# alanross/AlvaAR

Hardware: AMD Instinct MI355X
Metric: frames/sec @640x480 2000kp; local-BA residuals/sec (20KFx3k pts) (higher is better)
Workload: dtype u8/i16 image stages, f32 KLT, f64 pose+BA; 1 GPU; configs[1]: 640x480 RGBA stream, ~2000 keypoints/frame (cell 12), System::findCameraPose dataflow (fb-KLT -> P3P-LMedS -> PnP; keyframes: detect + describe, triangulate, map matching, local BA) via alva_system_find_camera_pose_device, steady state, frames resident in HBM; parallelism=1 independent camera streams, one per GPU, no collective on the data path

## Files before the change

alvaar_amd/csrc/image.hip:

```cpp
#include "common.hpp"
#include "multi_kernel.hpp"

namespace {

__device__ __forceinline__ uint32_t gray_of(uint32_t rgba) {
    uint32_t r = rgba & 0xff, g = (rgba >> 8) & 0xff, b = (rgba >> 16) & 0xff;
    return (9798u * r + 19235u * g + 3735u * b + 16384u) >> 15;
}

__device__ __forceinline__ void store_mirrors(uint8_t *g, size_t pitch, int w, int h, int win, int x, int y, uint8_t v) {
    int xs[3], ys[3];
    int nx = 0, ny = 0;
    xs[nx++] = x;
    if (x >= 1 && x <= win) xs[nx++] = -x;
    if (x <= w - 2 && x >= w - 1 - win) xs[nx++] = 2 * (w - 1) - x;
    ys[ny++] = y;
    if (y >= 1 && y <= win) ys[ny++] = -y;
    if (y <= h - 2 && y >= h - 1 - win) ys[ny++] = 2 * (h - 1) - y;
    if (nx == 1 && ny == 1) return;
    for (int j = 0; j < ny; j++)
        for (int i = 0; i < nx; i++)
            if (i | j) g[(ptrdiff_t) ys[j] * (ptrdiff_t) pitch + xs[i]] = v;
}

template<bool SRC_RGBA>
__device__ __forceinline__ void level0_body(const uint8_t *__restrict__ src, size_t src_pitch, int w, int h, int win,
                                            uint8_t *__restrict__ dst, size_t dst_pitch, uint8_t *__restrict__ gray_out,
                                            size_t gray_out_pitch, const int bx, const int by) {
    int x4 = (bx * 64 + threadIdx.x) * 4;
    int y = by * 4 + threadIdx.y;
    if (x4 >= w || y >= h) return;
    uint32_t packed;
    if (SRC_RGBA) {
        const uint4 p = *reinterpret_cast<const uint4 *>(src + (size_t) y * src_pitch + (size_t) x4 * 4);
        packed = gray_of(p.x) | (gray_of(p.y) << 8) | (gray_of(p.z) << 16) | (gray_of(p.w) << 24);
    } else {
        packed = *reinterpret_cast<const uint32_t *>(src + (size_t) y * src_pitch + x4);
    }
    *reinterpret_cast<uint32_t *>(dst + (size_t) y * dst_pitch + x4) = packed;
    if (gray_out) *reinterpret_cast<uint32_t *>(gray_out + (size_t) y * gray_out_pitch + x4) = packed;
// ... 108 lines not shown
    int acc[4] = {0, 0, 0, 0};
#pragma unroll
    for (int j = 0; j < 5; j++) {
        const uint8_t *row = a.g + (ptrdiff_t) (2 * y - 2 + j) * (ptrdiff_t) a.g_pitch + (2 * x - 4);
        const uint32_t *rp = reinterpret_cast<const uint32_t *>(row);
        const uint32_t w[4] = {rp[0], rp[1], rp[2], rp[3]};
        auto px = [&](int c) -> int { return (int) ((w[c >> 2] >> (8 * (c & 3))) & 0xffu); };
        const int wj = (j == 0 || j == 4) ? 1 : (j == 2 ? 6 : 4);
#pragma unroll
        for (int k = 0; k < 4; k++) {
            const int c0 = 2 + 2 * k;
            const int s = px(c0) + px(c0 + 4) + 4 * (px(c0 + 1) + px(c0 + 3)) + 6 * px(c0 + 2);
            acc[k] += wj * s;
        }
    }
    uint8_t out[4];
#pragma unroll
    for (int k = 0; k < 4; k++) out[k] = (uint8_t) ((acc[k] + 128) >> 8);
    uint8_t *dst = a.ng + (size_t) y * a.ng_pitch + x;
    if (x + 3 < a.dw) {
        *reinterpret_cast<uint32_t *>(dst) = (uint32_t) out[0] | ((uint32_t) out[1] << 8) | ((uint32_t) out[2] << 16) | ((uint32_t) out[3] << 24);
    } else {
        for (int k = 0; k < 4 && x + k < a.dw; k++) dst[k] = out[k];
    }
    for (int k = 0; k < 4 && x + k < a.dw; k++) store_mirrors(a.ng, a.ng_pitch, a.dw, a.dh, a.win, x + k, y, out[k]);
}

__host__ __device__ constexpr int rest_tile(int L) { return L == 3 ? 8 : 16; }
constexpr int R3 = 18;
constexpr int R2 = 23;
constexpr int R1 = 49;
constexpr int R0 = 101;
constexpr int R0P = (R0 + 3 + 3) / 4 * 4;
struct RestLevel {
    uint8_t *g;
    size_t g_pitch;
    int16_t *d;
    size_t d_pitch;
    int w, h;
};
struct RestArgs {
    StageArgs s0;
    RestLevel lv[4];
    int nlevels, win;
    int first[4], bx[4], ntiles[4];
    int ts[4];
};
struct Span {
    int lo, hi;
};
__device__ __forceinline__ int mirror101(int c, int n) { return c < 0 ? -c : (c >= n ? 2 * (n - 1) - c : c); }
__device__ __forceinline__ int mirror_in(int c, int n) { return min(max(mirror101(c, n), 0), n - 1); }
__device__ __forceinline__ Span below(Span s, int n) { return Span{2 * max(s.lo, 0) - 2, 2 * min(s.hi, n - 1) + 2}; }

__device__ __forceinline__ void down_tile(const uint8_t *src, int spitch, Span sx, Span sy, uint8_t *dst, int dpitch, Span dx, Span dy, int nx,
                                          int ny, int tid) {
    const int dw = dx.hi - dx.lo + 1, dh = dy.hi - dy.lo + 1;
    for (int e = tid; e < dw * dh; e += 256) {
        const int j = e / dw, i = e - j * dw;
        const int mx = mirror101(dx.lo + i, nx), my = mirror101(dy.lo + j, ny);
        const uint8_t *p = src + (2 * my - 2 - sy.lo) * spitch + (2 * mx - 2 - sx.lo);
        int acc = 0;
#pragma unroll
        for (int r = 0; r < 5; r++) {
            const uint8_t *q = p + r * spitch;
            const int srow = q[0] + q[4] + 4 * (q[1] + q[3]) + 6 * q[2];
            acc += ((r == 0 || r == 4) ? 1 : (r == 2 ? 6 : 4)) * srow;
        }
        dst[j * dpitch + i] = (uint8_t) ((acc + 128) >> 8);
    }
}

template<bool FROM_RGBA>
__device__ __forceinline__ void deep_tile(const RestArgs &A, int L, int bid, const uint8_t *__restrict__ rgba = nullptr, size_t rgba_pitch = 0) {
    __shared__ __attribute__((aligned(16))) uint8_t b0[R0 * R0P];
    __shared__ uint8_t b1[R1 * R1], b2[R2 * R2], b3[R3 * R3];
    const int tid = threadIdx.y * 64 + threadIdx.x;
    const RestLevel &T = A.lv[L];
    const int ts = A.ts[L];
    const int ox = (bid % A.bx[L]) * ts, oy = (bid / A.bx[L]) * ts;
    __shared__ Span sx[4], sy[4];
    if (tid == 0) {
        sx[L] = Span{ox - 1, min(ox + ts, T.w)};
        sy[L] = Span{oy - 1, min(oy + ts, T.h)};
        for (int l = L; l >= 1; l--) {
            sx[l - 1] = below(sx[l], A.lv[l].w);
            sy[l - 1] = below(sy[l], A.lv[l].h);
        }
    }
    __syncthreads();
    const RestLevel &Z = A.lv[0];
    const int xa = (sx[0].lo & ~3);
    const int ndw = (sx[0].hi - xa) / 4 + 1, nrow = sy[0].hi - sy[0].lo + 1;
    for (int e = tid; e < ndw * nrow; e += 256) {
        const int r = e / ndw, c = e - r * ndw;
        uint32_t v;
        if (FROM_RGBA) {
            const int yy = mirror_in(sy[0].lo + r, Z.h), x0 = xa + 4 * c;
            const uint8_t *rowp = rgba + (size_t) yy * rgba_pitch;
            if (x0 >= 0 && x0 + 3 < Z.w) {
                const uint4 p = *reinterpret_cast<const uint4 *>(rowp + 4 * (size_t) x0);
                v = gray_of(p.x) | (gray_of(p.y) << 8) | (gray_of(p.z) << 16) | (gray_of(p.w) << 24);
            } else {
                v = 0;
#pragma unroll
                for (int k = 0; k < 4; k++)
                    v |= gray_of(*reinterpret_cast<const uint32_t *>(rowp + 4 * (size_t) mirror_in(x0 + k, Z.w))) << (8 * k);
            }
        } else {
            v = *reinterpret_cast<const uint32_t *>(Z.g + (ptrdiff_t) (sy[0].lo + r) * (ptrdiff_t) Z.g_pitch + xa + 4 * c);
        }
        *reinterpret_cast<uint32_t *>(b0 + r * R0P + 4 * c) = v;
    }
    __syncthreads();
    const Span s0x{xa, sx[0].hi};
    Span px = s0x, py = sy[0];
    for (int l = 1; l <= L; l++) {
        const uint8_t *src = l == 1 ? b0 : (l == 2 ? b1 : b2);
        const int sp = l == 1 ? R0P : (l == 2 ? R1 : R2);
        uint8_t *dst = l == L ? b3 : (l == 1 ? b1 : b2);
        const int dp = l == L ? R3 : (l == 1 ? R1 : R2);
        down_tile(src, sp, px, py, dst, dp, sx[l], sy[l], A.lv[l].w, A.lv[l].h, tid);
        __syncthreads();
        px = sx[l];
        py = sy[l];
    }
    const int tx = tid % ts, ty = tid / ts;
    const int x = ox + tx, y = oy + ty;
    if (ty >= ts || x >= T.w || y >= T.h) return;
    const uint8_t *c = b3 + (ty + 1) * R3 + (tx + 1);
    const uint8_t v = c[0];
    T.g[(size_t) y * T.g_pitch + x] = v;
    store_mirrors(T.g, T.g_pitch, T.w, T.h, A.win, x, y, v);
    int t0[3], t1[3];
#pragma unroll
    for (int k = 0; k < 3; k++) {
        const int p0 = c[-R3 + k - 1], p1 = c[k - 1], p2 = c[R3 + k - 1];
        t0[k] = (p0 + p2) * 3 + p1 * 10;
        t1[k] = p2 - p0;
    }
    const short ix = (short) (t0[2] - t0[0]), iy = (short) ((t1[2] + t1[0]) * 3 + t1[1] * 10);
    int16_t *drow = reinterpret_cast<int16_t *>(reinterpret_cast<uint8_t *>(T.d) + (size_t) y * T.d_pitch) + 2 * x;
    *reinterpret_cast<uint32_t *>(drow) = (uint32_t) (uint16_t) ix | ((uint32_t) (uint16_t) iy << 16);
}

__device__ __forceinline__ void pyr_rest_body(const RestArgs &A, const int bid) {
    if (bid < A.s0.scharr_blocks) {
        scharr_tile(A.s0, bid);
        return;
    }
    int L = 1;
    while (L + 1 < A.nlevels && bid >= A.first[L + 1]) L++;
    const int n = A.ntiles[L];
    const int lb = bid - A.first[L], per = (n + 7) / 8;
    const int tile = (lb & 7) * per + (lb >> 3);
    if (tile >= n) return;
    deep_tile<false>(A, L, tile);
}
__global__ void __launch_bounds__(256) k_pyr_rest(RestArgs A) { pyr_rest_body(A, (int) blockIdx.x); }
ALVA_MULTI_KERNEL(MK_PYR_REST, k_pyr_rest_multi, RestArgs, dim3(64, 4), 256, pyr_rest_body(A, bx));

static int all_tile(int L, size_t pixels) {
    if (L == 3) return pixels <= 500000 ? 4 : 6;
    return L == 1 ? 16 : 12;
}
constexpr int L0_TW = 64, L0_TH = 16, L0_P = L0_TW + 8;
struct AllArgs {
    RestArgs R;
    const uint8_t *rgba;
    size_t rgba_pitch;
    uint8_t *gray_out;
    size_t gray_out_pitch;
    int l0_first, l0_bx;
};
__device__ __forceinline__ uint32_t gray4(const uint8_t *p) {
    const uint4 q = *reinterpret_cast<const uint4 *>(p);
    return gray_of(q.x) | (gray_of(q.y) << 8) | (gray_of(q.z) << 16) | (gray_of(q.w) << 24);
}
__device__ __forceinline__ void level0_tile(const AllArgs &A, const int tile) {
    __shared__ __attribute__((aligned(16))) uint8_t t[(L0_TH + 2) * L0_P];
    const int tid = threadIdx.y * 64 + threadIdx.x;
    const RestLevel &Z = A.R.lv[0];
    const int w = Z.w, h = Z.h, win = A.R.win;
    const int ox = (tile % A.l0_bx) * L0_TW, oy = (tile / A.l0_bx) * L0_TH;
    const int tx = tid & 15, ty = tid >> 4;
    const int x4 = ox + 4 * tx, y = oy + ty;
    const bool in = x4 < w && y < h;
    if (in) {
        const uint32_t packed = gray4(A.rgba + (size_t) y * A.rgba_pitch + (size_t) x4 * 4);
        *reinterpret_cast<uint32_t *>(t + (ty + 1) * L0_P + 4 + 4 * tx) = packed;
        *reinterpret_cast<uint32_t *>(Z.g + (size_t) y * Z.g_pitch + x4) = packed;
        if (A.gray_out) *reinterpret_cast<uint32_t *>(A.gray_out + (size_t) y * A.gray_out_pitch + x4) = packed;
        const bool edge_y = (y <= win) || (y >= h - 1 - win);
        const bool edge_x = (x4 <= win) || (x4 + 3 >= w - 1 - win);
        if (edge_x || edge_y) {
#pragma unroll
            for (int k = 0; k < 4; k++) store_mirrors(Z.g, Z.g_pitch, w, h, win, x4 + k, y, (uint8_t) (packed >> (8 * k)));
// ... 344 lines not shown
```

alvaar_amd/csrc/slam/frontend.cpp:

```cpp
#include "slam.hpp"
#if defined(__x86_64__)
#include <immintrin.h>
#endif
#include <chrono>
#include <cstdio>
#include <cmath>
#include <cstdlib>
#include <cstring>
#include <stdexcept>

namespace alva_slam {

namespace {
struct Section {
    double &acc;
    std::chrono::steady_clock::time_point t0 = std::chrono::steady_clock::now();
    explicit Section(double &a) : acc(a) {}
    ~Section() { acc += std::chrono::duration<double>(std::chrono::steady_clock::now() - t0).count(); }
};
}

Slam::Slam(Stages *stages, const Camera &c, const Settings &s) : st(stages), cam(c), cfg(s) {
    const float cw = std::ceil((float) cam.width / (float) cfg.cell_size), ch = std::ceil((float) cam.height / (float) cfg.cell_size);
    cfg.max_keypoints = (int) (cw * ch);
    camera_inverse_K(cam, invK);
    cur = std::make_shared<FrameRec>();
    cur->init(&cam, (size_t) cfg.cell_size);
    st->image_width_ = cam.width;
    st->image_height_ = cam.height;
    ba_arena_.assign((size_t) 4 << 20, 0);
    const char *chk = std::getenv("ALVA_CHECK_OBS_MIRROR");
    check_obs_mirror_ = chk && chk[0] == '1';
    const char *chk_carry = std::getenv("ALVA_CHECK_CARRY");
    check_carry_ = chk_carry && chk_carry[0] == '1';
}

void Slam::reset() {
    slots_dirty_ = true;
    cur->reset();
    st->reset_images();
    pose_failed = 0;
    next_mp_id = next_kf_id = n_map_points = n_keyframes = 0;
    map_generation++;
    keyframes.clear();
    for (auto e: map_points) destroy_map_point(e.second);
    map_points.clear();
    kf_flat_.clear();
    mp_flat_.clear();
    mp_rec_.clear();
    mp_slot_.clear();
    mp_nobs_.clear();
    mp_index_.clear();
    shared_ids.clear();
    ready_for_init = false;
    reset_requested = false;
    lost = false;
    reloc_lost_frames = 0;
}

int Slam::process_frame(const uint8_t *rgba, double timestamp, bool frame_on_device) {
    err_ = 0;
    cur->id++;
    cur->timestamp = timestamp;
    if (lost) return process_lost(rgba, timestamp, frame_on_device);
    track(rgba, timestamp, frame_on_device);
    fail(st->frame_done());
    if (err_) return err_;
    if (reset_requested) {
        reset();
        return 2;
    }
    if (!ready_for_init) return 3;
    if (lost) {
        cur->set_Twc(last_good_Twc_);
        return 4;
    }
    last_good_Twc_ = cur->Twc;
    return 1;
}

void Slam::enter_lost() {
    lost = true;
    reloc_lost_frames = 1;
    reloc_repack_ = true;
    reset_frame();
}
// ... 731 lines not shown
```

alvaar_amd/csrc/slam/map.cpp:

```cpp
#include "slam.hpp"
#if defined(__linux__)
#include <sys/mman.h>
#endif
#include <chrono>
#include <cmath>
#include <cstdio>
#include <cstdlib>
#include <cstring>
#include <limits>
#include <stdexcept>

namespace alva_slam {

namespace {
struct Lap {
    std::chrono::steady_clock::time_point t0 = std::chrono::steady_clock::now();
    void operator()(double &acc) {
        const auto t1 = std::chrono::steady_clock::now();
        acc += std::chrono::duration<double>(t1 - t0).count();
        t0 = t1;
    }
};
}

// ... 246 lines not shown
    if ((int) cur->n_kps > cfg.max_keypoints) {
        for (size_t ci = 0; ci < cur->grid.size(); ci++) {
            if (cur->grid[ci].size() <= 2) continue;
            const std::vector<int> ids = cur->grid[ci].to_vector();
            if (ids.size() > 2) {
                int to_remove = -1;
                size_t min_obs = std::numeric_limits<size_t>::max();
                bool broke = false;
                for (int lmid: ids) {
                    const MpRec *it = rec_raw(lmid);
                    if (it) {
                        const size_t nobs = it->n_obs;
                        if (nobs < min_obs) {
                            to_remove = lmid;
                            min_obs = nobs;
                        }
                    } else {
                        remove_obs_from_cur(lmid);
                        broke = true;
                        break;
                    }
                }
                (void) broke;
                if (to_remove >= 0) remove_obs_from_cur(to_remove);
            }
        }
    }
    ids_scratch_.clear();
    for (const auto &e: cur->kps)
        if (!rec_raw(e.first)) ids_scratch_.push_back(e.first);
    for (int id: ids_scratch_) remove_obs_from_cur(id);
}

void Slam::prepare_frame_observers() {
    const std::vector<int> &ids = kp_ids_;
    for (size_t i = 0; i < ids.size(); i++) {
        const int id = ids[i];
        prefetch_mp(ids.data(), i, ids.size());
        MpRec *r = rec_raw(id);
        if (!r) continue;
        ObsEnt *e = rec_slot(*r, next_kf_id);
        if (!e) {
            med_log.overflow = true;
            continue;
        }
        if (!(e->flags & MPF_OBS)) {
            e->flags |= MPF_OBS;
            r->n_obs++;
        }
        mp_nobs_[(size_t) id] = r->n_obs;
    }
}

void Slam::describe_tracked_begin() {
    const int n = (int) cur->kps.size();
    kp_ids_.clear();
    kp_pts_.resize((size_t) n * 2);
    kp_nodes_.resize((size_t) n);
    size_t i = 0;
    for (auto e: cur->kps) {
        kp_ids_.push_back(e.first);
        kp_nodes_[i] = &e.second;
        kp_pts_[2 * i] = e.second.px[0];
        kp_pts_[2 * i + 1] = e.second.px[1];
        i++;
    }
    if (n) fail(st->describe_begin(n, kp_pts_.data()));
}

void Slam::extract_keypoints() {
    if (err_) return;
    const int n = (int) kp_ids_.size();
    const std::vector<int> &kp_ids = kp_ids_;
    const std::vector<float> &pts = kp_pts_;
    const std::vector<KeyPt *> &nodes = kp_nodes_;
    const int to_detect = cfg.max_keypoints - (int) cur->n_occupied;
    const int cap = (int) cur->grid_cells + 8;
    std::vector<uint8_t> desc((size_t) n * 32), valid((size_t) n);
    if (n) {
        Lap lap;
        if (fail(st->describe_end(desc.data(), valid.data()))) return;
        lap(t_kf[1]);
    }
    Lap lap_det;
    if (to_detect > 0 && fail(st->detect_begin(cfg.cell_size, n, pts.data(), cap))) return;
    lap_det(t_kf[2]);
    if (n) {
        Lap lap;
        for (int i = 0; i < n; i++) {
            prefetch_mp_desc(kp_ids.data(), (size_t) i, (size_t) n);
            if (valid[(size_t) i]) {
                Desc d;
                __builtin_memcpy(d.b, &desc[(size_t) i * 32], 32);
                nodes[(size_t) i]->desc = d;
                nodes[(size_t) i]->has_desc = true;
                MapPt *mp = mp_raw(kp_ids[(size_t) i]);
                if (!mp) throw std::out_of_range("map point");
                mp->add_desc(cur->kfid, d);
            }
        }
        lap(t_kf[15]);
    }
    if (to_detect > 0) {
        std::vector<float> np((size_t) cap * 2);
        int count = 0;
        Lap lap;
        if (fail(st->detect_end(np.data(), &count))) return;
        lap(t_kf[2]);
        if (count > 0) {
            std::vector<uint8_t> desc((size_t) count * 32), valid((size_t) count);
            std::vector<float> unpx((size_t) count * 2);
            std::vector<double> bv((size_t) count * 3);
            if (fail(st->describe_and_compute(count, np.data(), desc.data(), valid.data(), unpx.data(), bv.data()))) return;
            lap(t_kf[3]);
            Lap fine;
            t_fine[26] += (double) count;
            for (int i = 0; i < count; i++) {
                KeyPt k;
                k.id = next_mp_id;
                k.px[0] = np[2 * (size_t) i]; k.px[1] = np[2 * (size_t) i + 1];
                k.unpx[0] = unpx[2 * (size_t) i]; k.unpx[1] = unpx[2 * (size_t) i + 1];
                for (int c = 0; c < 3; c++) k.bv[c] = bv[3 * (size_t) i + c];
                if (valid[(size_t) i]) {
                    __builtin_memcpy(k.desc.b, &desc[(size_t) i * 32], 32);
                    k.has_desc = true;
                    cur->add(k);
                    add_map_point(&k.desc);
                } else {
                    cur->add(k);
                    add_map_point(nullptr);
                }
            }
            fine(t_fine[13]);
        }
    }
}

void *alva_huge_alloc(size_t bytes) {
    const size_t huge = (size_t) 2 << 20, sz = (bytes + huge - 1) / huge * huge;
    void *p = std::aligned_alloc(huge, sz);
    if (!p) return nullptr;
#if defined(__linux__)
    static const bool off = std::getenv("ALVA_NO_HUGE_ARENA") != nullptr;
    if (!off) madvise(p, sz, MADV_HUGEPAGE);
#endif
    std::memset(p, 0, sz);
    return p;
}

Slam::~Slam() {
    if (chunk_ahead_.th.joinable()) chunk_ahead_.th.join();
}

void Slam::start_chunk_ahead(int index) {
    static const bool off = std::getenv("ALVA_NO_CHUNK_AHEAD") != nullptr;
    if (off || chunk_ahead_.th.joinable()) return;
    chunk_ahead_.index = index;
    chunk_ahead_.rec = nullptr;
    chunk_ahead_.dsc.reset();
    chunk_ahead_.keys.reset();
    chunk_ahead_.objs.reset();
    chunk_ahead_.th = std::thread([this, index] {
        chunk_ahead_.rec = st->mp_arena_chunk(index);
        chunk_ahead_.dsc = HugeArray<DescBlock>(MP_CHUNK);
// ... 25 lines not shown
        if (!dsc) dsc = HugeArray<DescBlock>(MP_CHUNK);
        if (!keys) keys = HugeArray<DescKeys>(MP_CHUNK);
        if (!objs) objs = HugeArray<MapPtBox>(MP_CHUNK);
        if (!dsc || !keys || !objs) return false;
        med_log.chunks.push_back(chunk);
        med_log.desc_chunks.push_back(std::move(dsc));
        med_log.key_chunks.push_back(std::move(keys));
        mp_obj_chunks_.push_back(std::move(objs));
        static const bool timing = std::getenv("ALVA_ARENA_TIMING") != nullptr;
        if (timing)
            std::fprintf(stderr, "[arena] chunk %d: %.0f us\n", index, 1e6 * std::chrono::duration<double>(std::chrono::steady_clock::now() - t0).count());
        start_chunk_ahead(index + 1);
    }
    return true;
}

const ObsEnt *Slam::obs_of(const MapPt &mp, int kfid) const {
    const ObsEnt *o = mp.in_kf(kfid);
    if (check_obs_mirror_) {
        const FrameRec *kf = kf_raw(kfid);
        const KeyPt *kp = kf ? kf->find(mp.id()) : nullptr;
        if ((kp != nullptr) != (o != nullptr) || (kp && (std::memcmp(kp->px, o->px, 8) || std::memcmp(kp->unpx, o->unpx, 8)))) {
            std::fprintf(stderr, "alva_slam: observation mirror out of sync (map point %d, keyframe %d)\n", mp.id(), kfid);
            std::abort();
        }
    }
    return o;
}

void Slam::add_keyframe() {
    Lap fine;
    std::shared_ptr<FrameRec> kf = std::make_shared<FrameRec>(*cur);
    fine(t_fine[10]);
    for (const auto &e: kf->kps) {
        MapPt *m = mp_raw(e.first);
        if (m) m->note_px(next_kf_id, e.second);
    }
    fine(t_fine[12]);
    keyframes.emplace(next_kf_id, kf);
    if (kf_flat_.size() <= (size_t) next_kf_id) kf_flat_.resize((size_t) next_kf_id + 32, nullptr);
    kf_flat_[(size_t) next_kf_id] = kf.get();
    n_keyframes++;
    next_kf_id++;
}

void Slam::add_map_point(const Desc *d) {
    const int slot = med_log.alloc();
    if (!ensure_rec_chunk(slot)) {
        med_log.release(slot);
        fail(-3);
        return;
    }
    MapPt *mp = d ? new (mp_box_fresh(slot)) MapPt(&med_log, slot, next_mp_id, next_kf_id, *d) : new (mp_box_fresh(slot)) MapPt(&med_log, slot, next_mp_id, next_kf_id);
    map_points.insert_slot(next_mp_id, mp);
    if (mp_flat_.size() <= (size_t) next_mp_id) {
        mp_flat_.resize((size_t) next_mp_id + 4096, nullptr);
        mp_rec_.resize(mp_flat_.size(), nullptr);
        mp_slot_.resize(mp_flat_.size(), -1);
        mp_nobs_.resize(mp_flat_.size(), 0);
    }
    mp_flat_[(size_t) next_mp_id] = mp;
    mp_rec_[(size_t) next_mp_id] = mp->r;
    mp_slot_[(size_t) next_mp_id] = slot;
    sync_nobs(*mp);
    next_mp_id++;
    n_map_points++;
}

void Slam::update_map_point(int id, const double *wpt, double anchor_inv_depth) {
    MpRec *rec = rec_raw(id);
    if (!rec) return;
    mp_edits_++;
    if (rec->is3d) {
        rec->X[0] = wpt[0]; rec->X[1] = wpt[1]; rec->X[2] = wpt[2];
        if (anchor_inv_depth >= 0.) rec->inv_depth = anchor_inv_depth;
        return;
    }
    MapPt &mp = *mp_raw(id);
    if (!mp.r->is3d) {
        const ObsList obs = mp.observers();
        for (int kf: obs) {
            FrameRec *k = kf_raw(kf);
            if (k) k->turn3d(id);
            else mp.remove_obs(kf);
        }
        sync_nobs(mp);
        if (mp.r->observed) cur->turn3d(id);
    }
    mp.r->X[0] = wpt[0]; mp.r->X[1] = wpt[1]; mp.r->X[2] = wpt[2];
    mp.r->is3d = 1;
    if (anchor_inv_depth >= 0.) mp.r->inv_depth = anchor_inv_depth;
}

void Slam::merge_map_points(int prev_id, int new_id) {
    MapPt *prev = mp_raw(prev_id), *nw = mp_raw(new_id);
    if (!prev || !nw || !nw->r->is3d) return;
    const ObsList next_kfs = nw->observers(), prev_kfs = prev->observers();
    const DescKeys prev_desc = prev->kf_desc;
    for (int pk: prev_kfs) {
        auto kf = keyframes.find(pk);
        if (kf == keyframes.end()) continue;
        if (kf->second->change_id(prev_id, new_id, nw->r->is3d != 0)) {
            prev->drop_px(pk);
            nw->note_px(pk, *kf->second->find(new_id));
            nw->obs_insert(pk);
            sync_nobs(*nw);
            for (int nk: next_kfs) {
                auto co = keyframes.find(nk);
                if (co != keyframes.end()) {
                    kf->second->add_covisible(nk);
                    co->second->add_covisible(pk);
                }
            }
        }
    }
    for (int se = prev_desc.first(); se != DescKeys::END; se = prev_desc.next(se)) {
        const uint8_t *b = prev->dsc[se];
        Desc d;
        std::memcpy(d.b, b, 32);
        nw->add_desc(prev_desc.key(se), d);
    }
    if (cur->observes(prev_id)) {
        if (cur->change_id(prev_id, new_id, nw->r->is3d != 0)) set_map_point_obs(new_id);
    }
    if (prev->r->is3d) n_map_points--;
    {
        auto sh = shared_ids.find(prev_id);
        if (sh != shared_ids.end()) {
            shared_ids.emplace(new_id, sh->second);
            shared_ids.erase(sh);
        }
    }
    mp_flat_[(size_t) prev_id] = nullptr;
    mp_rec_[(size_t) prev_id] = nullptr;
    mp_slot_[(size_t) prev_id] = -1;
    mp_nobs_[(size_t) prev_id] = 0;
    map_points.erase(prev_id);
    destroy_map_point(prev);
    n_merges++;
}

void Slam::remove_keyframe(int kfid) {
    auto it = keyframes.find(kfid);
    if (it == keyframes.end()) return;
    std::vector<int> &ids = rm_ids_;
    ids.clear();
    it->second->for_each_id([&](int kid, bool) { ids.push_back(kid); });
    for (size_t i = 0; i < ids.size(); i++) {
        prefetch_mp_desc(ids.data(), i, ids.size());
        MapPt *m = mp_raw(ids[i]);
        if (m) {
            m->remove_obs(kfid);
            m->drop_px(kfid);
            sync_nobs(*m);
        }
    }
    for (const auto &c: it->second->covisible) {
        auto co = keyframes.find(c.first);
        if (co != keyframes.end()) co->second->remove_covisible(kfid);
    }
    kf_flat_[(size_t) kfid] = nullptr;
    keyframes.erase(it);
    n_keyframes--;
}

void Slam::remove_map_point(int id) {
    MapPt *mp = mp_raw(id);
    if (!mp) return;
    const ObsList obs = mp->observers();
    for (int kf: obs) {
        auto k = keyframes.find(kf);
        if (k == keyframes.end()) continue;
        k->second->remove(id);
        for (int co: obs)
            if (co != kf) k->second->decrease_covisible(co);
    }
    if (mp->r->observed) cur->remove(id);
    if (mp->r->is3d) n_map_points--;
    mp_flat_[(size_t) id] = nullptr;
    mp_rec_[(size_t) id] = nullptr;
    mp_slot_[(size_t) id] = -1;
    mp_nobs_[(size_t) id] = 0;
    map_points.erase(id);
    if (defer_mp_free_) mp_graveyard_.push_back(mp);
    else destroy_map_point(mp);
}

void Slam::remove_map_point_obs(int mp_id, int kfid) {
    auto kf = keyframes.find(kfid);
    if (kf != keyframes.end()) kf->second->remove(mp_id);
    MapPt *m = mp_raw(mp_id);
    if (!m) return;
    m->drop_px(kfid);
    m->remove_obs(kfid);
    sync_nobs(*m);
    if (kf != keyframes.end()) {
        const ObsList obs = m->observers();
        for (int co: obs) {
            auto c = keyframes.find(co);
            if (c != keyframes.end()) {
                kf->second->decrease_covisible(co);
                c->second->decrease_covisible(kfid);
            }
        }
    }
}

void Slam::remove_obs_from_cur(int mp_id) {
    cur->remove(mp_id);
    MpRec *m = rec_raw(mp_id);
    if (!m) return;
    m->observed = 0;
}

bool Slam::set_map_point_obs(int mp_id) {
    MpRec *m = rec_raw(mp_id);
    if (!m) return false;
    m->observed = 1;
    return true;
}

void Slam::update_frame_covisibility(FrameRec &frame) {
    Lap fine;
    std::map<int, int> cov;
    FlatSet local_ids;
    ids_scratch_.clear();
    for (const auto &e: frame.kps) ids_scratch_.push_back(e.first);
    std::vector<int> &count = index_scratch_;
    count.assign((size_t) next_kf_id + 2, 0);
    for (size_t oi = 0; oi < ids_scratch_.size(); oi++) {
        const int id = ids_scratch_[oi];
        prefetch_mp(ids_scratch_.data(), oi, ids_scratch_.size());
        const MpRec *m = rec_raw(id);
        if (!m) {
            remove_map_point_obs(id, frame.kfid);
            remove_obs_from_cur(id);
            continue;
        }
        for (int e = 0; e < m->n_ent; e++) {
            if (!(m->ent[e].flags & MPF_OBS)) continue;
            const int kf = m->ent[e].kf;
            if (kf != frame.kfid) {
                if (kf >= 0 && kf <= next_kf_id) count[(size_t) kf]++;
                else cov[kf] += 1;
            }
        }
    }
    for (int kf = 0; kf <= next_kf_id; kf++)
        if (count[(size_t) kf]) cov[kf] += count[(size_t) kf];
    fine(t_fine[14]);
    std::set<int> bad;
    mark_a_.resize((size_t) next_mp_id + 1, 0);
    mark_b_.resize((size_t) next_mp_id + 1, 0);
    touched_a_.clear();
    touched_b_.clear();
    for (const auto &e: frame.kps) {
        mark_a_[(size_t) e.first] = 1;
        touched_a_.push_back(e.first);
    }
    kf_ptrs_.clear();
    for (const auto &c: cov) kf_ptrs_.push_back(kf_raw(c.first));
    FrameRec::refresh_ids3d(kf_ptrs_.data(), kf_ptrs_.size());
    for (const auto &c: cov) {
        FrameRec *kf = kf_raw(c.first);
        if (kf) {
            kf->covisible[frame.kfid] = c.second;
            const std::vector<int> &ids = kf->ids3d();
            if (fresh_ids_.size() < ids.size() + 1) fresh_ids_.resize(ids.size() + 1);
            int *fresh = fresh_ids_.data();
            size_t nf = 0;
            const uint8_t *ma = mark_a_.data(), *mb = mark_b_.data();
            for (int kid: ids) {
                fresh[nf] = kid;
                nf += (size_t) !(ma[(size_t) kid] | mb[(size_t) kid]);
            }
            for (size_t i = 0; i < nf; i++) {
                const int kid = fresh[i];
                mark_b_[(size_t) kid] = 1;
                touched_b_.push_back(kid);
                local_ids.insert_new(kid);
            }
        } else {
// ... 16 lines not shown
```

alvaar_amd/csrc/slam/slam.hpp:

```cpp
#pragma once
#if defined(__SANITIZE_ADDRESS__)
#include <sanitizer/asan_interface.h>
#endif
#include <cstdlib>
#include <new>
#include <map>
#include <memory>
#include <memory_resource>
#include <set>
#include <thread>
#include <unordered_map>
#include <unordered_set>
#include <vector>
#include "flat_hash.hpp"
#include "mp_rec.hpp"
#include "se3.hpp"
#include "stages.hpp"

namespace alva_slam {

struct Desc {
    uint8_t b[32];
};

// ... 469 lines not shown
    int par_frame_ = -1, par_kfid_ = -1;
    void prepare_parallax();
    float parallax_of_pairs(const FrameRec &kf);
    float median_of_distinct(std::vector<uint32_t> &all);
    std::vector<int> ids_scratch_, obs_scratch_, index_scratch_, mp_index_, kf_ids_scratch_, local_scratch_, rm_ids_;
    std::vector<uint8_t> mark_a_, mark_b_;
    std::vector<int> touched_a_, touched_b_;
    bool fail(int rc) { if (rc && !err_) err_ = rc; return rc != 0; }
    SE3 last_good_Twc_;
    bool reloc_repack_ = true;
    std::vector<int> reloc_slot_, reloc_id_;
    std::vector<double> reloc_wpt_;
    void enter_lost();
    int process_lost(const uint8_t *rgba, double timestamp, bool frame_on_device);

    bool track(const uint8_t *rgba, double timestamp, bool frame_on_device);
    bool process(double timestamp);
    void klt_from_motion_prior();
    bool compute_pose();
    float compute_parallax(int kfid, bool unrotate, bool median);
    bool check_ready_for_init();
    bool check_new_keyframe_required();
    void reset_frame();
    void apply_motion_model(SE3 &Twc, double time);
    void update_motion_model(const SE3 &Twc, double time);

    void create_keyframe();
    void prepare_frame_removals();
    void describe_tracked_begin();
    void prepare_frame_observers();
    std::vector<int> kp_ids_;
    std::vector<float> kp_pts_;
    std::vector<KeyPt *> kp_nodes_;
    void extract_keypoints();
    void add_keyframe();
    void add_map_point(const Desc *d);
    void update_map_point(int id, const double *wpt, double anchor_inv_depth);
public:
    void merge_map_points(int prev_id, int new_id);
private:
    void remove_keyframe(int kfid);
    void remove_map_point(int id);
    void remove_map_point_obs(int mp_id, int kfid);
    void remove_obs_from_cur(int mp_id);
    bool set_map_point_obs(int mp_id);
    void update_frame_covisibility(FrameRec &frame);
    std::shared_ptr<FrameRec> keyframe(int id) const;
    void prefetch_tables(int id) const {
        if (id >= 0 && (size_t) id < mp_rec_.size()) {
            __builtin_prefetch(&mp_rec_[(size_t) id]);
            __builtin_prefetch(&mp_slot_[(size_t) id]);
        }
    }
    void prefetch_mp(const int *ids, size_t i, size_t n, size_t far_d = 10) const {
        if (i + 2 * far_d < n) prefetch_tables(ids[i + 2 * far_d]);
        if (i + far_d < n) {
            const MpRec *f = rec_raw(ids[i + far_d]);
            if (f) {
                const char *c = (const char *) f;
                __builtin_prefetch(c);
                __builtin_prefetch(c + 64);
                __builtin_prefetch(c + 128);
                __builtin_prefetch(c + 192);
            }
        }
    }
    void prefetch_mp_desc(const int *ids, size_t i, size_t n, size_t near_d = 4, size_t far_d = 10) const {
        if (i + 2 * far_d < n) {
            const int id = ids[i + 2 * far_d];
// ... 91 lines not shown
```

alvaar_amd/system.py:

```python
from __future__ import annotations

import ctypes as C
import math
import os

import numpy as np

from .capi import lib, AlvaError

_vp, _i, _d = C.c_void_p, C.c_int, C.c_double
lib.alva_system_create.argtypes = [_i, C.POINTER(_vp)]
lib.alva_system_destroy.argtypes = [_vp]
lib.alva_system_destroy.restype = None
lib.alva_system_configure.argtypes = [_vp, _i, _i] + [_d] * 8
lib.alva_system_reset.argtypes = [_vp]
lib.alva_system_reset.restype = None
lib.alva_system_find_camera_pose.argtypes = [_vp, _vp, _vp]
lib.alva_system_find_camera_pose_with_imu.argtypes = [_vp, _vp, _vp, _vp]
lib.alva_system_find_camera_pose_with_imu_ts.argtypes = [_vp, _vp, _vp, C.c_double, _vp]
lib.alva_system_find_plane.argtypes = [_vp, _vp, _i]
lib.alva_system_get_frame_points.argtypes = [_vp, _vp]
lib.alva_system_get_keypoints.argtypes = [_vp, _vp, _vp, _vp, _i]
lib.alva_system_configure_ex.argtypes = [_vp, _i, _i] + [_d] * 8 + [_i] * 3
lib.alva_system_find_camera_pose_ts.argtypes = [_vp, _vp, _d, _vp]
# ... 668 lines not shown
        if n < 0:
            raise AlvaError(lib.alva_system_last_error().decode())
        n = min(n, cap)
        return a[:n], b[:n], c[:n]

    def counters(self):
        out = (C.c_long * 3)()
        lib.alva_system_debug_counters(self.h, out)
        return dict(ba_solves=out[0], merges=out[1], culled_keyframes=out[2])

    def klt_work(self, reset: bool = True):
        out = (C.c_long * 2)()
        lib.alva_system_debug_klt_work(self.h, out, int(reset))
        return int(out[0]), int(out[1])

    def timing(self, reset: bool = True):
        out = np.zeros(8)
        lib.alva_system_debug_timing(self.h, out.ctypes.data, int(reset))
        names = ("upload+pyramid", "gather", "track_step", "track_apply", "pose_wait", "pose_apply+kf_check", "keyframe_create", "mapping")
        return dict(zip(names, out))

    def timing_keyframe(self, reset: bool = True):
        out = np.zeros(16)
        lib.alva_system_debug_timing_keyframe(self.h, out.ctypes.data, int(reset))
        names = ("prepare", "describe_tracked", "detect", "describe_new", "insert+copy", "triangulate", "covisibility", "local_map_matching",
                 "optimize", "(match stage)", "(BA stage)", "(BA build)", "(BA solves+sweep)", "(BA write-back)", "(BA culling)", "(descriptor medoids)")
        return dict(zip(names, out[:16]))

    FINE_NAMES = ("match: local-map union", "match: flatten+stage", "match: merges", "flatten: kf table + cells", "flatten: local list",
                  "flatten: per map point", "BA build: keyframes + point set", "BA build: observations", "filter: keyframe removals",
                  "window: remove kf-30", "copy: frame", "copy: order mirror", "copy: observation mirror", "new keypoints + map points",
                  "covis: counts", "covis: local ids", "covis: into local map", "parallax pairs (all frames)", "parallax (all frames)", "parallax sort (all frames)",
                  "#flattened map points", "#flattened observations", "#local candidates", "#BA points", "#BA residual blocks", "#BA keyframes",
                  "#new keypoints", "#local ids", "#covisible keyframes", "#frames: slot table carried", "#frames: slot table assembled", "probe 31")

    def timing_fine(self, reset: bool = True):
        out = np.zeros(32)
        lib.alva_system_debug_timing_fine(self.h, out.ctypes.data, int(reset))
        return {n: v for n, v in zip(self.FINE_NAMES, out) if n}

    def set_init_pose(self, pose7):
        if pose7 is None:
            lib.alva_system_debug_set_init_pose(self.h, None)
        else:
            p = np.ascontiguousarray(pose7, np.float64)
            lib.alva_system_debug_set_init_pose(self.h, p.ctypes.data)


class SystemGroup:

    def __init__(self, sessions, n_threads: int):
        h = _vp()
        rc = lib.alva_system_group_create(int(n_threads), C.byref(h))
        if rc:
            raise AlvaError("alva_system_group_create failed")
        self.h = h
        self.set_sessions(sessions)

    def stream(self, index: int, device: int = 0):
        st = _vp()
        if lib.alva_system_group_stream(self.h, device, index, C.byref(st)):
            raise AlvaError("alva_system_group_stream failed")
        return st

    def set_lockstep(self, on: bool):
        if lib.alva_system_group_set_lockstep(self.h, 1 if on else 0):
            raise AlvaError("alva_system_group_set_lockstep failed")
# ... 43 lines not shown
```

Measured before the change: 4169 frames/s.

## Separate pyramid downsample into packed column and row passes with cheaper index math

The 5x5 pyramid downsample inside deep_tile is split into two passes. A vertical pass builds packed 16-bit column sums in shared memory, two pixels per dword, and a horizontal pass then reads them, which replaces the per-output 25-tap byte gather. Grayscale conversion now uses udot4 dot-product instructions, divisions are replaced by 24-bit multiply-shift reciprocals, RGBA loads are batched four deep for more memory-level parallelism, and the all_tile sizes change for small images. In exchange it adds an extra shared buffer and barrier per level, and it relies on the reciprocal division being exact for the small index ranges involved.

Result: no change. 4187 frames/s, median of 2 (+0.4%).

```diff
diff --git a/alvaar_amd/csrc/image.hip b/alvaar_amd/csrc/image.hip
--- a/alvaar_amd/csrc/image.hip
+++ b/alvaar_amd/csrc/image.hip
@@ -4,8 +4,9 @@
 namespace {
 
 __device__ __forceinline__ uint32_t gray_of(uint32_t rgba) {
-    uint32_t r = rgba & 0xff, g = (rgba >> 8) & 0xff, b = (rgba >> 16) & 0xff;
-    return (9798u * r + 19235u * g + 3735u * b + 16384u) >> 15;
+    const uint32_t hi = __builtin_amdgcn_udot4(rgba, 0x000e4b26u, 0u, false);
+    const uint32_t lo = __builtin_amdgcn_udot4(rgba, 0x00972346u, 16384u, false);
+    return ((hi << 8) + lo) >> 15;
 }
 
 __device__ __forceinline__ void store_mirrors(uint8_t *g, size_t pitch, int w, int h, int win, int x, int y, uint8_t v) {
@@ -180,6 +181,9 @@
 constexpr int R1 = 49;
 constexpr int R0 = 101;
 constexpr int R0P = (R0 + 3 + 3) / 4 * 4;
+constexpr int R1P = (R1 + 3) / 4 * 4;
+constexpr int R2P = (R2 + 3) / 4 * 4;
+constexpr int HP = R0P;
 struct RestLevel {
     uint8_t *g;
     size_t g_pitch;
@@ -201,28 +205,61 @@
 __device__ __forceinline__ int mirror_in(int c, int n) { return min(max(mirror101(c, n), 0), n - 1); }
 __device__ __forceinline__ Span below(Span s, int n) { return Span{2 * max(s.lo, 0) - 2, 2 * min(s.hi, n - 1) + 2}; }
 
-__device__ __forceinline__ void down_tile(const uint8_t *src, int spitch, Span sx, Span sy, uint8_t *dst, int dpitch, Span dx, Span dy, int nx,
-                                          int ny, int tid) {
+__device__ __forceinline__ uint32_t mul24(uint32_t a, uint32_t b) {
+    uint32_t d;
+    asm("v_mul_u32_u24_e32 %0, %1, %2" : "=v"(d) : "v"(a), "v"(b));
+    return d;
+}
+struct Div {
+    uint32_t m;
+    int n;
+    __device__ __forceinline__ explicit Div(int n_) : m((1u << 18) / (uint32_t) n_ + 1u), n(n_) {}
+    __device__ __forceinline__ int quot(int e) const { return (int) (mul24((uint32_t) e, m) >> 18); }
+    __device__ __forceinline__ int rem(int e, int q) const { return e - (int) mul24((uint32_t) q, (uint32_t) n); }
+};
+
+template<int SP>
+__device__ __forceinline__ void down_level(const uint8_t *src, Span sx, int sy_lo, uint16_t *cs, uint8_t *dst, int dpitch, Span dx, Span dy,
+                                           int nx, int ny, int tid) {
+    static_assert(SP % 4 == 0 && SP <= HP, "dword rows; the column sums of a source row fit a row of cs");
     const int dw = dx.hi - dx.lo + 1, dh = dy.hi - dy.lo + 1;
+    const int ndw = (sx.hi - sx.lo) / 4 + 1;
+    const Div by_ndw(ndw);
+    for (int e = tid; e < ndw * dh; e += 256) {
+        const int j = by_ndw.quot(e), c = by_ndw.rem(e, j);
+        const int my = mirror101(dy.lo + j, ny);
+        const uint32_t *p = reinterpret_cast<const uint32_t *>(src + mul24((uint32_t) (2 * my - 2 - sy_lo), SP)) + c;
+        uint32_t ev = 0, od = 0;
+#pragma unroll
+        for (int r = 0; r < 5; r++) {
+            const uint32_t v = p[r * (SP / 4)];
+            const uint32_t wr = (r == 0 || r == 4) ? 1u : (r == 2 ? 6u : 4u);
+            ev += wr * (v & 0x00ff00ffu);
+            od += wr * ((v >> 8) & 0x00ff00ffu);
+        }
+        uint2 o;
+        o.x = (ev & 0xffffu) | (od << 16);
+        o.y = (ev >> 16) | (od & 0xffff0000u);
+        *reinterpret_cast<uint2 *>(cs + j * HP + 4 * c) = o;
+    }
+    __syncthreads();
+    const Div by_dw(dw);
     for (int e = tid; e < dw * dh; e += 256) {
-        const int j = e / dw, i = e - j * dw;
-        const int mx = mirror101(dx.lo + i, nx), my = mirror101(dy.lo + j, ny);
-        const uint8_t *p = src + (2 * my - 2 - sy.lo) * spitch + (2 * mx - 2 - sx.lo);
-        int acc = 0;
-#pragma unroll
-        for (int r = 0; r < 5; r++) {
-            const uint8_t *q = p + r * spitch;
-            const int srow = q[0] + q[4] + 4 * (q[1] + q[3]) + 6 * q[2];
-            acc += ((r == 0 || r == 4) ? 1 : (r == 2 ? 6 : 4)) * srow;
-        }
-        dst[j * dpitch + i] = (uint8_t) ((acc + 128) >> 8);
-    }
+        const int j = by_dw.quot(e), i = by_dw.rem(e, j);
+        const int mx = mirror101(dx.lo + i, nx);
+        const uint32_t *q = reinterpret_cast<const uint32_t *>(cs + j * HP + (2 * mx - 2 - sx.lo));
+        const uint32_t a = q[0], b = q[1], c = q[2];
+        const uint32_t acc = (a & 0xffffu) + (c & 0xffffu) + 4u * ((a >> 16) + (b >> 16)) + mul24(b & 0xffffu, 6u);
+        dst[mul24((uint32_t) j, (uint32_t) dpitch) + i] = (uint8_t) ((acc + 128u) >> 8);
+    }
+    __syncthreads();
 }
 
 template<bool FROM_RGBA>
 __device__ __forceinline__ void deep_tile(const RestArgs &A, int L, int bid, const uint8_t *__restrict__ rgba = nullptr, size_t rgba_pitch = 0) {
-    __shared__ __attribute__((aligned(16))) uint8_t b0[R0 * R0P];
-    __shared__ uint8_t b1[R1 * R1], b2[R2 * R2], b3[R3 * R3];
+    __shared__ __attribute__((aligned(16))) uint8_t b0[R0 * R0P], b1[R1 * R1P], b2[R2 * R2P];
+    __shared__ __attribute__((aligned(16))) uint16_t cs[R1 * HP];
+    __shared__ uint8_t b3[R3 * R3];
     const int tid = threadIdx.y * 64 + threadIdx.x;
     const RestLevel &T = A.lv[L];
     const int ts = A.ts[L];
@@ -240,40 +277,48 @@
     const RestLevel &Z = A.lv[0];
     const int xa = (sx[0].lo & ~3);
     const int ndw = (sx[0].hi - xa) / 4 + 1, nrow = sy[0].hi - sy[0].lo + 1;
-    for (int e = tid; e < ndw * nrow; e += 256) {
-        const int r = e / ndw, c = e - r * ndw;
-        uint32_t v;
-        if (FROM_RGBA) {
-            const int yy = mirror_in(sy[0].lo + r, Z.h), x0 = xa + 4 * c;
-            const uint8_t *rowp = rgba + (size_t) yy * rgba_pitch;
-            if (x0 >= 0 && x0 + 3 < Z.w) {
-                const uint4 p = *reinterpret_cast<const uint4 *>(rowp + 4 * (size_t) x0);
-                v = gray_of(p.x) | (gray_of(p.y) << 8) | (gray_of(p.z) << 16) | (gray_of(p.w) << 24);
-            } else {
-                v = 0;
-#pragma unroll
-                for (int k = 0; k < 4; k++)
-                    v |= gray_of(*reinterpret_cast<const uint32_t *>(rowp + 4 * (size_t) mirror_in(x0 + k, Z.w))) << (8 * k);
+    constexpr int NB = 4;
+    const Div by_ndw(ndw);
+    const int total = ndw * nrow;
+    for (int e0 = tid; e0 < total; e0 += NB * 256) {
+        uint4 p[NB];
+        int at[NB];
+#pragma unroll
+        for (int k = 0; k < NB; k++) {
+            const int e = e0 + 256 * k;
+            at[k] = -1;
+            if (e < total) {
+                const int r = by_ndw.quot(e), c = by_ndw.rem(e, r);
+                at[k] = r * R0P + 4 * c;
+                if (FROM_RGBA) {
+                    const int yy = mirror_in(sy[0].lo + r, Z.h), x0 = xa + 4 * c;
+                    const uint8_t *rowp = rgba + (size_t) yy * rgba_pitch;
+                    if (x0 >= 0 && x0 + 3 < Z.w) {
+                        p[k] = *reinterpret_cast<const uint4 *>(rowp + 4 * (size_t) x0);
+                    } else {
+                        p[k].x = *reinterpret_cast<const uint32_t *>(rowp + 4 * (size_t) mirror_in(x0, Z.w));
+                        p[k].y = *reinterpret_cast<const uint32_t *>(rowp + 4 * (size_t) mirror_in(x0 + 1, Z.w));
+                        p[k].z = *reinterpret_cast<const uint32_t *>(rowp + 4 * (size_t) mirror_in(x0 + 2, Z.w));
+                        p[k].w = *reinterpret_cast<const uint32_t *>(rowp + 4 * (size_t) mirror_in(x0 + 3, Z.w));
+                    }
+                } else {
+                    p[k].x = *reinterpret_cast<const uint32_t *>(Z.g + (ptrdiff_t) (sy[0].lo + r) * (ptrdiff_t) Z.g_pitch + xa + 4 * c);
+                }
             }
-        } else {
-            v = *reinterpret_cast<const uint32_t *>(Z.g + (ptrdiff_t) (sy[0].lo + r) * (ptrdiff_t) Z.g_pitch + xa + 4 * c);
-        }
-        *reinterpret_cast<uint32_t *>(b0 + r * R0P + 4 * c) = v;
+        }
+#pragma unroll
+        for (int k = 0; k < NB; k++) {
+            if (at[k] < 0) continue;
+            const uint32_t v = FROM_RGBA ? gray_of(p[k].x) | (gray_of(p[k].y) << 8) | (gray_of(p[k].z) << 16) | (gray_of(p[k].w) << 24) : p[k].x;
+            *reinterpret_cast<uint32_t *>(b0 + at[k]) = v;
+        }
     }
     __syncthreads();
-    const Span s0x{xa, sx[0].hi};
-    Span px = s0x, py = sy[0];
-    for (int l = 1; l <= L; l++) {
-        const uint8_t *src = l == 1 ? b0 : (l == 2 ? b1 : b2);
-        const int sp = l == 1 ? R0P : (l == 2 ? R1 : R2);
-        uint8_t *dst = l == L ? b3 : (l == 1 ? b1 : b2);
-        const int dp = l == L ? R3 : (l == 1 ? R1 : R2);
-        down_tile(src, sp, px, py, dst, dp, sx[l], sy[l], A.lv[l].w, A.lv[l].h, tid);
-        __syncthreads();
-        px = sx[l];
-        py = sy[l];
-    }
-    const int tx = tid % ts, ty = tid / ts;
+    down_level<R0P>(b0, Span{xa, sx[0].hi}, sy[0].lo, cs, L == 1 ? b3 : b1, L == 1 ? R3 : R1P, sx[1], sy[1], A.lv[1].w, A.lv[1].h, tid);
+    if (L >= 2) down_level<R1P>(b1, sx[1], sy[1].lo, cs, L == 2 ? b3 : b2, L == 2 ? R3 : R2P, sx[2], sy[2], A.lv[2].w, A.lv[2].h, tid);
+    if (L >= 3) down_level<R2P>(b2, sx[2], sy[2].lo, cs, b3, R3, sx[3], sy[3], A.lv[3].w, A.lv[3].h, tid);
+    const Div by_ts(ts);
+    const int ty = by_ts.quot(tid), tx = by_ts.rem(tid, ty);
     const int x = ox + tx, y = oy + ty;
     if (ty >= ts || x >= T.w || y >= T.h) return;
     const uint8_t *c = b3 + (ty + 1) * R3 + (tx + 1);
@@ -309,8 +354,8 @@
 ALVA_MULTI_KERNEL(MK_PYR_REST, k_pyr_rest_multi, RestArgs, dim3(64, 4), 256, pyr_rest_body(A, bx));
 
 static int all_tile(int L, size_t pixels) {
-    if (L == 3) return pixels <= 500000 ? 4 : 6;
-    return L == 1 ? 16 : 12;
+    if (pixels > 500000) return rest_tile(L);
+    return L == 3 ? 4 : (L == 2 ? 12 : 16);
 }
 constexpr int L0_TW = 64, L0_TH = 16, L0_P = L0_TW + 8;
 struct AllArgs {
```

## Fold keyframe covisibility counting into observer preparation and note pixels inline

Applied to the files above, without the earlier changes.

Covisibility counts are now accumulated incrementally while the new keyframe's observers are prepared, and kept consistent through point removal and observation removal. The later covisibility pass reuses that table instead of rescanning every map point record, and falls back to the full scan when a merge or a missing record makes the table inexact. Keypoint pixels are written into the observation entries during preparation and when a map point is created, replacing the per-keypoint note_px loop in add_keyframe, and keyframe scratch vectors are reused across calls. This adds bookkeeping hooks to several removal paths, which must stay exactly in sync with the record state.

New measurement: 4195 frames/s before, 4186 frames/s after, median of 2. Within noise of the previous version (-0.2%).

```diff
diff --git a/alvaar_amd/csrc/slam/frontend.cpp b/alvaar_amd/csrc/slam/frontend.cpp
--- a/alvaar_amd/csrc/slam/frontend.cpp
+++ b/alvaar_amd/csrc/slam/frontend.cpp
@@ -33,6 +33,8 @@
     check_obs_mirror_ = chk && chk[0] == '1';
     const char *chk_carry = std::getenv("ALVA_CHECK_CARRY");
     check_carry_ = chk_carry && chk_carry[0] == '1';
+    const char *chk_fold = std::getenv("ALVA_CHECK_KF_FOLD");
+    check_kf_fold_ = check_obs_mirror_ || (chk_fold && chk_fold[0] == '1');
 }
 
 void Slam::reset() {
@@ -52,6 +54,9 @@
     mp_nobs_.clear();
     mp_index_.clear();
     shared_ids.clear();
+    cov_.kf = -1;
+    cov_.mark.clear();
+    cov_.marked.clear();
     ready_for_init = false;
     reset_requested = false;
     lost = false;
diff --git a/alvaar_amd/csrc/slam/map.cpp b/alvaar_amd/csrc/slam/map.cpp
--- a/alvaar_amd/csrc/slam/map.cpp
+++ b/alvaar_amd/csrc/slam/map.cpp
@@ -302,14 +302,58 @@
     for (int id: ids_scratch_) remove_obs_from_cur(id);
 }
 
+void Slam::cov_begin() {
+    for (int id: cov_.marked)
+        if ((size_t) id < cov_.mark.size()) cov_.mark[(size_t) id] = 0;
+    cov_.marked.clear();
+    cov_.mark.resize((size_t) next_mp_id + 1, 0);
+    cov_.count.assign((size_t) next_kf_id + 2, 0);
+    cov_.kf = next_kf_id;
+    cov_.inexact = false;
+}
+
+void Slam::cov_point_leaves(int mp_id) {
+    if (!cov_counted(mp_id)) return;
+    cov_.mark[(size_t) mp_id] = 0;
+    const MpRec *r = rec_raw(mp_id);
+    if (!r) {
+        cov_.inexact = true;
+        return;
+    }
+    for (int e = 0; e < r->n_ent; e++)
+        if ((r->ent[e].flags & MPF_OBS) && r->ent[e].kf != cov_.kf) cov_add(r->ent[e].kf, -1);
+}
+
+void Slam::mp_remove_obs(MapPt &m, int kf) {
+    if (kf != cov_.kf && cov_counted(m.id()) && m.obs_has(kf)) cov_add(kf, -1);
+    m.remove_obs(kf);
+}
+
 void Slam::prepare_frame_observers() {
     const std::vector<int> &ids = kp_ids_;
+    cov_begin();
+    int *count = cov_.count.data();
+    const int kfid = next_kf_id;
     for (size_t i = 0; i < ids.size(); i++) {
         const int id = ids[i];
         prefetch_mp(ids.data(), i, ids.size());
+        if (i + 3 < ids.size()) {
+            const MpRec *f = rec_raw(ids[i + 3]);
+            if (f)
+                for (size_t off = 256, end = sizeof(MpRec) - sizeof(f->ent) + (size_t) (f->n_ent + 1) * sizeof(ObsEnt); off < end && off < sizeof(MpRec); off += 64)
+                    __builtin_prefetch((const char *) f + off, 1);
+        }
         MpRec *r = rec_raw(id);
-        if (!r) continue;
-        ObsEnt *e = rec_slot(*r, next_kf_id);
+        if (!r) {
+            cov_.inexact = true;
+            continue;
+        }
+        const int n_ent = r->n_ent;
+        if (n_ent && (r->ent[0].kf < 0 || r->ent[n_ent - 1].kf > kfid)) cov_.inexact = true;
+        else
+            for (int k = 0; k < n_ent; k++) count[r->ent[k].kf] += r->ent[k].flags & MPF_OBS;
+        cov_.mark[(size_t) id] = 1;
+        ObsEnt *e = rec_slot(*r, kfid);
         if (!e) {
             med_log.overflow = true;
             continue;
@@ -318,8 +362,14 @@
             e->flags |= MPF_OBS;
             r->n_obs++;
         }
+        const KeyPt &k = *kp_nodes_[i];
+        e->flags |= MPF_INKF;
+        e->px[0] = k.px[0]; e->px[1] = k.px[1];
+        e->unpx[0] = k.unpx[0]; e->unpx[1] = k.unpx[1];
         mp_nobs_[(size_t) id] = r->n_obs;
     }
+    count[kfid] = 0;
+    cov_.marked = ids;
 }
 
 void Slam::describe_tracked_begin() {
@@ -346,7 +396,10 @@
     const std::vector<KeyPt *> &nodes = kp_nodes_;
     const int to_detect = cfg.max_keypoints - (int) cur->n_occupied;
     const int cap = (int) cur->grid_cells + 8;
-    std::vector<uint8_t> desc((size_t) n * 32), valid((size_t) n);
+    KfScratch &S = kf_scratch_;
+    std::vector<uint8_t> &desc = S.desc, &valid = S.valid;
+    desc.resize((size_t) n * 32);
+    valid.resize((size_t) n);
     if (n) {
         Lap lap;
         if (fail(st->describe_end(desc.data(), valid.data()))) return;
@@ -372,15 +425,20 @@
         lap(t_kf[15]);
     }
     if (to_detect > 0) {
-        std::vector<float> np((size_t) cap * 2);
+        std::vector<float> &np = S.np;
+        np.resize((size_t) cap * 2);
         int count = 0;
         Lap lap;
         if (fail(st->detect_end(np.data(), &count))) return;
         lap(t_kf[2]);
         if (count > 0) {
-            std::vector<uint8_t> desc((size_t) count * 32), valid((size_t) count);
-            std::vector<float> unpx((size_t) count * 2);
-            std::vector<double> bv((size_t) count * 3);
+            std::vector<uint8_t> &desc = S.new_desc, &valid = S.new_valid;
+            std::vector<float> &unpx = S.unpx;
+            std::vector<double> &bv = S.bv;
+            desc.resize((size_t) count * 32);
+            valid.resize((size_t) count);
+            unpx.resize((size_t) count * 2);
+            bv.resize((size_t) count * 3);
             if (fail(st->describe_and_compute(count, np.data(), desc.data(), valid.data(), unpx.data(), bv.data()))) return;
             lap(t_kf[3]);
             Lap fine;
@@ -394,12 +452,9 @@
                 if (valid[(size_t) i]) {
                     __builtin_memcpy(k.desc.b, &desc[(size_t) i * 32], 32);
                     k.has_desc = true;
-                    cur->add(k);
-                    add_map_point(&k.desc);
-                } else {
-                    cur->add(k);
-                    add_map_point(nullptr);
                 }
+                cur->add(k);
+                add_map_point(k);
             }
             fine(t_fine[13]);
         }
@@ -491,9 +546,21 @@
     Lap fine;
     std::shared_ptr<FrameRec> kf = std::make_shared<FrameRec>(*cur);
     fine(t_fine[10]);
-    for (const auto &e: kf->kps) {
-        MapPt *m = mp_raw(e.first);
-        if (m) m->note_px(next_kf_id, e.second);
+    if (check_kf_fold_) {
+        for (const auto &e: kf->kps) {
+            MapPt *m = mp_raw(e.first);
+            if (!m) continue;
+            const int i = rec_find(*m->r, next_kf_id);
+            ObsEnt before;
+            if (i >= 0) before = m->r->ent[i];
+            m->note_px(next_kf_id, e.second);
+            const int j = rec_find(*m->r, next_kf_id);
+            if (med_log.overflow) continue;
+            if (i < 0 || j != i || std::memcmp(&before, &m->r->ent[j], sizeof(ObsEnt))) {
+                std::fprintf(stderr, "alva_slam: keyframe %d: the pixel of map point %d was not noted with its observer\n", next_kf_id, e.first);
+                std::abort();
+            }
+        }
     }
     fine(t_fine[12]);
     keyframes.emplace(next_kf_id, kf);
@@ -503,7 +570,8 @@
     next_kf_id++;
 }
 
-void Slam::add_map_point(const Desc *d) {
+void Slam::add_map_point(const KeyPt &k) {
+    const Desc *d = k.has_desc ? &k.desc : nullptr;
     const int slot = med_log.alloc();
     if (!ensure_rec_chunk(slot)) {
         med_log.release(slot);
@@ -521,6 +589,7 @@
     mp_flat_[(size_t) next_mp_id] = mp;
     mp_rec_[(size_t) next_mp_id] = mp->r;
     mp_slot_[(size_t) next_mp_id] = slot;
+    mp->note_px(next_kf_id, k);
     sync_nobs(*mp);
     next_mp_id++;
     n_map_points++;
@@ -541,7 +610,7 @@
         for (int kf: obs) {
             FrameRec *k = kf_raw(kf);
             if (k) k->turn3d(id);
-            else mp.remove_obs(kf);
+            else mp_remove_obs(mp, kf);
         }
         sync_nobs(mp);
         if (mp.r->observed) cur->turn3d(id);
@@ -554,6 +623,7 @@
 void Slam::merge_map_points(int prev_id, int new_id) {
     MapPt *prev = mp_raw(prev_id), *nw = mp_raw(new_id);
     if (!prev || !nw || !nw->r->is3d) return;
+    if (cov_.kf >= 0) cov_.inexact = true;
     const ObsList next_kfs = nw->observers(), prev_kfs = prev->observers();
     const DescKeys prev_desc = prev->kf_desc;
     for (int pk: prev_kfs) {
@@ -609,7 +679,7 @@
         prefetch_mp_desc(ids.data(), i, ids.size());
         MapPt *m = mp_raw(ids[i]);
         if (m) {
-            m->remove_obs(kfid);
+            mp_remove_obs(*m, kfid);
             m->drop_px(kfid);
             sync_nobs(*m);
         }
@@ -626,6 +696,7 @@
 void Slam::remove_map_point(int id) {
     MapPt *mp = mp_raw(id);
     if (!mp) return;
+    cov_point_leaves(id);
     const ObsList obs = mp->observers();
     for (int kf: obs) {
         auto k = keyframes.find(kf);
@@ -647,11 +718,14 @@
 
 void Slam::remove_map_point_obs(int mp_id, int kfid) {
     auto kf = keyframes.find(kfid);
-    if (kf != keyframes.end()) kf->second->remove(mp_id);
+    if (kf != keyframes.end()) {
+        if (kfid == cov_.kf) cov_point_leaves(mp_id);
+        kf->second->remove(mp_id);
+    }
     MapPt *m = mp_raw(mp_id);
     if (!m) return;
     m->drop_px(kfid);
-    m->remove_obs(kfid);
+    mp_remove_obs(*m, kfid);
     sync_nobs(*m);
     if (kf != keyframes.end()) {
         const ObsList obs = m->observers();
@@ -685,28 +759,50 @@
     FlatSet local_ids;
     ids_scratch_.clear();
     for (const auto &e: frame.kps) ids_scratch_.push_back(e.first);
+    const bool folded = cov_.kf == frame.kfid && !cov_.inexact;
+    if (!folded) t_fine[31] += 1.;
     std::vector<int> &count = index_scratch_;
-    count.assign((size_t) next_kf_id + 2, 0);
-    for (size_t oi = 0; oi < ids_scratch_.size(); oi++) {
-        const int id = ids_scratch_[oi];
-        prefetch_mp(ids_scratch_.data(), oi, ids_scratch_.size());
-        const MpRec *m = rec_raw(id);
-        if (!m) {
+    if (folded && !check_kf_fold_) {
+        for (int id: ids_scratch_) {
+            if (rec_raw(id)) continue;
             remove_map_point_obs(id, frame.kfid);
             remove_obs_from_cur(id);
-            continue;
-        }
-        for (int e = 0; e < m->n_ent; e++) {
-            if (!(m->ent[e].flags & MPF_OBS)) continue;
-            const int kf = m->ent[e].kf;
-            if (kf != frame.kfid) {
-                if (kf >= 0 && kf <= next_kf_id) count[(size_t) kf]++;
-                else cov[kf] += 1;
-            }
-        }
-    }
-    for (int kf = 0; kf <= next_kf_id; kf++)
-        if (count[(size_t) kf]) cov[kf] += count[(size_t) kf];
+        }
+    } else {
+        count.assign((size_t) next_kf_id + 2, 0);
+        for (size_t oi = 0; oi < ids_scratch_.size(); oi++) {
+            const int id = ids_scratch_[oi];
+            prefetch_mp(ids_scratch_.data(), oi, ids_scratch_.size());
+            const MpRec *m = rec_raw(id);
+            if (!m) {
+                remove_map_point_obs(id, frame.kfid);
+                remove_obs_from_cur(id);
+                continue;
+            }
+            for (int e = 0; e < m->n_ent; e++) {
+                if (!(m->ent[e].flags & MPF_OBS)) continue;
+                const int kf = m->ent[e].kf;
+                if (kf != frame.kfid) {
+                    if (kf >= 0 && kf <= next_kf_id) count[(size_t) kf]++;
+                    else cov[kf] += 1;
+                }
+            }
+        }
+        if (folded) {
+            for (int kf = 0; kf <= next_kf_id; kf++) {
+                const int acc = (size_t) kf < cov_.count.size() ? cov_.count[(size_t) kf] : 0;
+                if (acc != count[(size_t) kf] || !cov.empty()) {
+                    std::fprintf(stderr, "alva_slam: keyframe %d: covisibility with keyframe %d accumulated as %d, counted as %d\n", frame.kfid, kf,
+                                 acc, count[(size_t) kf]);
+                    std::abort();
+                }
+            }
+        }
+    }
+    const std::vector<int> &table = folded ? cov_.count : count;
+    for (int kf = 0; kf <= next_kf_id && (size_t) kf < table.size(); kf++)
+        if (table[(size_t) kf]) cov[kf] += table[(size_t) kf];
+    cov_.kf = -1;
     fine(t_fine[14]);
     std::set<int> bad;
     mark_a_.resize((size_t) next_mp_id + 1, 0);
diff --git a/alvaar_amd/csrc/slam/slam.hpp b/alvaar_amd/csrc/slam/slam.hpp
--- a/alvaar_amd/csrc/slam/slam.hpp
+++ b/alvaar_amd/csrc/slam/slam.hpp
@@ -525,9 +525,30 @@
     std::vector<int> kp_ids_;
     std::vector<float> kp_pts_;
     std::vector<KeyPt *> kp_nodes_;
+    struct KfScratch {
+        std::vector<uint8_t> desc, valid, new_desc, new_valid;
+        std::vector<float> np, unpx;
+        std::vector<double> bv;
+    } kf_scratch_;
+    struct CovFold {
+        int kf = -1;
+        bool inexact = false;
+        std::vector<int> count;
+        std::vector<uint8_t> mark;
+        std::vector<int> marked;
+    } cov_;
+    bool check_kf_fold_ = false;
+    void cov_begin();
+    bool cov_counted(int mp_id) const { return cov_.kf >= 0 && mp_id >= 0 && (size_t) mp_id < cov_.mark.size() && cov_.mark[(size_t) mp_id]; }
+    void cov_add(int kf, int d) {
+        if (kf >= 0 && (size_t) kf < cov_.count.size()) cov_.count[(size_t) kf] += d;
+        else cov_.inexact = true;
+    }
+    void cov_point_leaves(int mp_id);
+    void mp_remove_obs(MapPt &m, int kf);
     void extract_keypoints();
     void add_keyframe();
-    void add_map_point(const Desc *d);
+    void add_map_point(const KeyPt &k);
     void update_map_point(int id, const double *wpt, double anchor_inv_depth);
 public:
     void merge_map_points(int prev_id, int new_id);
diff --git a/alvaar_amd/system.py b/alvaar_amd/system.py
--- a/alvaar_amd/system.py
+++ b/alvaar_amd/system.py
@@ -724,7 +724,8 @@
                   "window: remove kf-30", "copy: frame", "copy: order mirror", "copy: observation mirror", "new keypoints + map points",
                   "covis: counts", "covis: local ids", "covis: into local map", "parallax pairs (all frames)", "parallax (all frames)", "parallax sort (all frames)",
                   "#flattened map points", "#flattened observations", "#local candidates", "#BA points", "#BA residual blocks", "#BA keyframes",
-                  "#new keypoints", "#local ids", "#covisible keyframes", "#frames: slot table carried", "#frames: slot table assembled", "probe 31")
+                  "#new keypoints", "#local ids", "#covisible keyframes", "#frames: slot table carried", "#frames: slot table assembled",
+                  "#keyframes: covisibility counted from the records")
 
     def timing_fine(self, reset: bool = True):
         out = np.zeros(32)
```
